# AdrienCorenflos/aux-ssm-samplers

Hardware: AMD Instinct MI355X
Metric: Gibbs sweeps/sec (aux-Kalman, parallel-in-time scan) (higher is better)
Workload: dtype f64; 1 GPU; C2: linear-Gaussian SSM T=65536 d=4 p=8, aux-Kalman sweep, parallel scan; chains_per_gpu=256, parallelism=chains x1 (independent, no collective)

## Files before the change

### aux_ssm_samplers_amd/csrc/api.hip

```cpp
#include <cstdarg>
#include <cstdlib>
#include <cstring>

#include "ctx.h"
#include "rng.h"

namespace ax {

static thread_local std::string g_err;
void set_error(const char* fmt, ...) {
    char buf[1024];
    va_list ap;
    va_start(ap, fmt);
    vsnprintf(buf, sizeof buf, fmt, ap);
    va_end(ap);
    g_err = buf;
}

int ws_reserve(auxssm_ctx* h, size_t bytes) {
    h->ws_off = 0;
    if (bytes <= h->ws_bytes) return AUXSSM_OK;
    if (h->ws) {
        AX_HIP(hipStreamSynchronize(h->stream));
        AX_HIP(hipFree(h->ws));
// ... 672 lines not shown
    if (aux_fly) {
        set_aux_fly(fa, c, 1, xA, epsauxA, uA);
        if (gen) fa.aux_gen = 1, fa.gen_k0 = keys[0], fa.gen_k1 = keys[1];
    }
    if (wide_shared) {
        const long long tot = (long long)T * P;
        hipLaunchKernelGGL((k_concat_carrier<R>), dim3((unsigned)((tot + 255) / 256)), dim3(256), 0, h->stream, T, D, P, cv(*c.yobs), carrier);
        fa.mask_ys = Arr{carrier, 0, (long long)P, 0, 1};
    }
    rc = ke->filter(h, fa, parallel, ell);
    if (rc) return rc;
    h->ws_off = mark;
    SampleArgs sa;
    fill_sample_args(sa, kd, D, cv(model->Fs), cv(model->Qs), cv(model->bs), msA, PsA, epsA, xpA, cm);
    sa.ps_shared = shared_mode ? 1 : 0;
    sa.ps_packed = ps_pack ? 1 : 0;
    if (gen) sa.eps_gen = 1, sa.gen_k0 = keys[2], sa.gen_k1 = keys[3];
    rc = se->sample(h, sa, parallel);
    if (rc) return rc;
    h->ws_off = mark;

    SweepLogpdfArgs la;
    fill_sweep_logpdf_args(la, c, kd, *model, cv(*c.yobs), xA, xpA, uA, aux_fly ? 1 : 0, epsauxA);
    rc = sl->run(h, la, sums);
    if (rc) return rc;
    h->ws_off = mark;
    launch_accept<R>(c, sums, ell, ell);
    if ((rc = launch_select<R>(h, C, T, D, (const int32_t*)c.accepted, xpA, xA, cm))) return rc;
    AX_HIP(hipGetLastError());
    return AUXSSM_OK;
}

template <typename R>
__global__ void k_fs_concat0(int C, int D, int PO, const R* __restrict__ xa, const R* __restrict__ xb, const int32_t* __restrict__ sel, const R* __restrict__ eps0, R shd,
                             const double* dptr, Arr yobs, R* __restrict__ u, R* __restrict__ ysc0) {
    if (dptr) shd = (R)dptr[1];
    const int P = D + PO;
    const int g = blockIdx.x * blockDim.x + threadIdx.x;
    if (g >= C * P) return;
    const int c = g % C, k = g / C;
    if (k < D) {
        const R* x = (sel && sel[c]) ? xb : xa;
        const R v = x[(long long)k * C + c] + shd * eps0[(long long)k * C + c];
        u[(long long)k * C + c] = v;
        ysc0[(long long)k * C + c] = v;
    } else {
        ysc0[(long long)k * C + c] = at<R>(yobs, 0, 0, 0)[k - D];
    }
}
template <typename R> __global__ void __launch_bounds__(256) k_fs_resolve(int C, const int32_t* __restrict__ sel, const R* __restrict__ xb, R* __restrict__ xa) {
    const int c = blockIdx.y * 256 + threadIdx.x;
    if (c >= C) return;
    const long long off = (long long)blockIdx.x * C + c;
    if (sel[c]) xa[off] = xb[off];
}
template <typename R>
__global__ void __launch_bounds__(256) k_fs_stats(int C, const int32_t* __restrict__ accepted, const int32_t* __restrict__ sel, const R* __restrict__ xa, const R* __restrict__ xb,
                                                   R* __restrict__ sq_jump, R* __restrict__ mean, R* __restrict__ sq_mean, long long iter) {
    const int c = blockIdx.y * 256 + threadIdx.x;
    if (c >= C) return;
    const long long off = (long long)blockIdx.x * C + c;
    const int s = sel[c], acc = accepted[c];
    const R xn = (s ? xb : xa)[off];
    const R xo = acc ? (s ? xa : xb)[off] : xn;
    const R it = (R)iter, dj = xn - xo;
    sq_jump[off] = fold_mean<R>(it, sq_jump[off], dj * dj);
    mean[off] = fold_mean<R>(it, mean[off], xn);
    sq_mean[off] = fold_mean<R>(it, sq_mean[off], xn * xn);
}
static const char* fused_refusal(const auxssm_ctx* h, const auxssm_dims* dims, const auxssm_lgssm* model, int parallel, int layout) {
    const int C = dims->C, T = dims->T, D = dims->dx, PO = dims->dy;
    if (layout != AUXSSM_LAYOUT_CHAIN_MINOR) return "the fused sweep takes the chain-minor layout";
    if (D > MAX_D || PO < 1 || PO > 4) return "the fused sweep is instantiated for dx <= 4, 1 <= dy <= 4";
    if (!parallel) return "the fused sweep is the parallel-in-time one";
    if (!h->share_model) return "AUXSSM_OPT_SHARE_MODEL is off";
    if (!prior_chain_shared(model)) return "the fused sweep needs chain-shared model parameters (chain stride 0)";
    if (C < 2 || (C % 2) != 0) return "the fused sweep pairs chains for its in-kernel draws: the chain count must be even";
    if (T < 64) return "the fused sweep needs T >= 64";
    return nullptr;
}
template <typename R> static int sweep_lg_concat_fused(const SweepCall& c) {
    auxssm_ctx* h = c.h;
    const auxssm_lgssm* model = c.model;
    const auxssm_arr* yobs = c.yobs;
    const double delta = c.delta;
    void *x = c.x, *x_alt = c.x_alt;
    const int C = c.dims->C, T = c.dims->T, D = c.dims->dx, PO = c.dims->dy, P = D + PO;
    const SweepLogpdfEntry* sl = sweep_logpdf_entry(c.dtype, D, PO);
    if (!sl || !sl->fused) {
        set_error("(dx=%d, dy=%d) has no fused sweep in this build", D, PO);
        return AUXSSM_ERR_UNSUPPORTED;
    }
    const KDims kd{C, T, 1};
    const size_t sR = sizeof(R), CT = (size_t)C * T;
    const size_t stage[4] = {(size_t)T * P * D * sR, (size_t)T * P * P * sR, (size_t)T * P * sR, (size_t)T * D * D * sR};
    R *u, *inc, *ysc0, *m0p, *eps0a, *eps0s;
    WsPlan ws;
    ws.add(u, CT * D * sR);
    ws.add(inc, CT * D * sR);
    ws.add(ysc0, (size_t)C * P * sR);
    ws.add(m0p, (size_t)C * D * sR);
    ws.add(eps0a, (size_t)C * D * sR);
    ws.add(eps0s, (size_t)C * D * sR);
    for (size_t b : stage) ws.after(b);
    ws.after(sl->fused_ws(h, kd));
    int rc = ws.reserve(h);
    if (rc) return rc;
    bool overlap = h->overlap_model_stage != 0 && !c.dptr;
    SweepEnd sweep_end{h};
    if (overlap) {
        const size_t need_side = sl->fused_ws(h, kd) + (size_t)(T + 64) * sR * ((size_t)P * D + (size_t)P * P + P + (size_t)D * D) + (4u << 20) +
                                 (size_t)(T + 2) * sR * (3 * (size_t)D * D + 2 * D + (size_t)PO * D + (size_t)PO * PO + 2 * PO);
        if ((rc = side_open(h, need_side))) return rc;
        overlap = h->side.open;
    }
    const bool tinv = obs_model_time_invariant(model);
    const int* memo = nullptr;
    struct MemoGuard {
        auxssm_ctx* h;
        int p = -1;
        bool ok = false;
        ~MemoGuard() { if (p >= 0 && !ok) h->side.memo_use[p] = -1; }
    } memo_guard{h};
    if (overlap) {
        SideScope sc(h);
        auxssm_ctx::SideStage& sd = h->side;
        const int p = sd.parity;
        MemoDesc md{};
        const auxssm_arr* srcs[9] = {&model->m0, &model->P0, &model->Fs, &model->Qs, &model->bs, &model->Hs, &model->Rs, &model->cs, yobs};
        const int recs[9] = {D, D * D, D * D, D * D, D, PO * D, PO * PO, PO, PO};
        const int nts[9] = {1, 1, T - 1, T - 1, T - 1, T, T, T, T};
        md.n = 9;
        md.off[0] = 0;
        bool plain = true;
        for (int q = 0; q < 9; ++q) {
// ... 9 lines not shown
        if (plain) {
            std::vector<unsigned char> key;
            auto put = [&](const void* v, size_t nb) { key.insert(key.end(), (const unsigned char*)v, (const unsigned char*)v + nb); };
            const int hdr[8] = {(int)sR, C, T, D, PO, c.nan_policy, 0, 0};
            put(hdr, sizeof(hdr));
            put(&delta, sizeof(delta));
            for (int q = 0; q < 9; ++q) put(srcs[q], sizeof(auxssm_arr));
            const bool chain_ok = sd.memo_use[p] == sd.uses[p] - 1 && sd.memo_key[p] == key;
            const unsigned gmemo = (unsigned)std::min<long long>(1024, (md.off[9] + 255) / 256);
            if (chain_ok) {
                hipLaunchKernelGGL(k_memo_set, dim3(1), dim3(1), 0, h->stream, rebuild, 0);
                hipLaunchKernelGGL((k_memo_check<R>), dim3(gmemo), dim3(256), 0, h->stream, md, (const R*)snap, rebuild);
            } else {
                hipLaunchKernelGGL(k_memo_set, dim3(1), dim3(1), 0, h->stream, rebuild, 1);
            }
            hipLaunchKernelGGL((k_memo_snap<R>), dim3(gmemo), dim3(256), 0, h->stream, md, snap, (const int*)rebuild);
            sd.memo_key[p] = std::move(key);
            sd.memo_use[p] = sd.uses[p];
            memo_guard.p = p;
            memo = rebuild;
        }
    }
    R *Hc, *Rc, *cc, *Ps;
    ConcatModel cmod;
    {
        SideScope sc(h);
        Hc = (R*)ws_take(h, stage[0]);
        Rc = (R*)ws_take(h, stage[1]);
        cc = (R*)ws_take(h, stage[2]);
        Ps = (R*)ws_take(h, stage[3]);
        if (!Hc || !Rc || !cc || !Ps) return AUXSSM_ERR_NOMEM;
        cmod = concat_model<R>(c, tinv, Hc, Rc, cc, memo, nullptr);
    }
    launch_rng_sweep<R>(h, c.keys, (long long)D * C, C, eps0a, eps0s, const_cast<void*>(c.u_acc));
    hipLaunchKernelGGL((k_fs_concat0<R>), dim3((unsigned)((C * P + 255) / 256)), dim3(256), 0, h->stream, C, D, PO, (const R*)x, (const R*)x_alt, (const int32_t*)c.sel,
                       (const R*)eps0a, (R)c.shd(), c.dptr, cv(*yobs), u, ysc0);
    FusedHost f{};
    const KDims k1{C, 1, 1};
    const Arr none{};
    sweep_filter_args(f.fa, cmod.d, cmod.g, cm_arr(ysc0, k1, P), cm_arr(m0p, k1, D), Arr{Ps, 0, (long long)D * D, 0, 1}, 1);
    f.fa.pblk = D;
    set_aux_fly(f.fa, c, 1, none, none, none);
    fill_sample_args(f.sa, kd, D, cv(model->Fs), cv(model->Qs), cv(model->bs), none, f.fa.Ps, none, none, 1);
    f.sa.ps_shared = 1;
    fill_sweep_logpdf_args(f.la, c, kd, *model, cv(*yobs), cm_arr(x, kd, D), cm_arr(x_alt, kd, D), cm_arr(u, kd, D), 0, none);
    f.memo = memo;
    f.xa = x; f.xb = x_alt; f.sel = c.sel; f.u = u; f.inc = inc; f.keys = c.keys; f.eps0s = eps0s; f.u_acc = c.u_acc; f.accepted = c.accepted; f.logs = c.logs;
    if (h->st_mean && (h->st_x != x || h->st_n != (long long)C * T * D || h->st_dtype != (sizeof(R) == 4 ? AUXSSM_F32 : AUXSSM_F64))) {
        set_error("running moments are attached to another state (x=%p, n=%lld, dtype=%d): detach them (auxssm_stats_attach with NULLs) "
                  "before sweeping a different state on this handle", h->st_x, h->st_n, h->st_dtype);
        return AUXSSM_ERR_ARG;
    }
    if ((rc = sl->fused(h, f))) return rc;
    if (!c.sel) {
        if ((rc = launch_select<R>(h, C, T, D, (const int32_t*)c.accepted, cm_arr(x_alt, kd, D), cm_arr(x, kd, D), 1))) return rc;
    } else if (h->st_mean) {
        ProfScope ps(h, AUXSSM_K_SELECT);
        const long long rows = (long long)T * D;
        hipLaunchKernelGGL((k_fs_stats<R>), dim3((unsigned)rows, (unsigned)((C + 255) / 256)), dim3(256), 0, h->stream, C, (const int32_t*)c.accepted, (const int32_t*)c.sel,
                           (const R*)x, (const R*)x_alt, (R*)h->st_sq_jump, (R*)h->st_mean, (R*)h->st_sq_mean, h->st_iter);
        ++h->st_iter;
    }
    AX_HIP(hipGetLastError());
    memo_guard.ok = true;
    return AUXSSM_OK;
}

template <typename R> AX_HD R sv_nan_to_num(R v) { return nan_to_num<R>(v); }
template <typename R>
// ... 962 lines not shown
```

### aux_ssm_samplers_amd/csrc/fused_shared.h

```cpp
#pragma once

struct FusedArgs {
    int C, T, E, nchunk;
    const void* xa;
    void* xb;
    const int32_t* sel;
    void* u;
    void* inc;
    const void* gain;
    const void* samp;
    const void* logt;
    const void* gpre;
    const void* m0p;
    void* agg_f; void* pre_f; void* agg_s; void* pre_s;
    Acc* pa;
    Acc* pe;
    void* pell;
    const Acc* clog;
    const int* nanrow;
    unsigned ka0, ka1, ks0, ks1;
    const void* eps0s;
    double delta, shd;
    const double* dptr;
    int nan_policy;
// ... 52 lines not shown
#pragma unroll
        for (int k = 0; k < D * D; ++k) G[k] = row[TS::oG + k];
        mm<R, D, D, D>(M, G, o);
#pragma unroll
        for (int k = 0; k < D * D; ++k) M[k] = o[k];
    }
#pragma unroll
    for (int k = 0; k < D * D; ++k) cprod[(long long)(a.nchunk - 1 - ch) * D * D + k] = M[k];
}

template <typename R, int D> __global__ void __launch_bounds__(TB_CM) k_fs_psi(FusedArgs a, const R* __restrict__ gpre, const R* __restrict__ fpre, R* __restrict__ ntab,
                                                                              R* __restrict__ psi) {
    if (memo_skip(a)) return;
    using TS = SampShared<R, D>;
    const int ch = blockIdx.x * TB_CM + threadIdx.x;
    if (ch >= a.nchunk) return;
    const int t0 = ch * a.E, tb = min(a.T, t0 + a.E);
    R Ps[D * D];
#pragma unroll
    for (int k = 0; k < D * D; ++k) Ps[k] = 0;
    for (int t = t0; t < tb; ++t) {
        const R* row = (const R*)a.samp + (long long)t * TS::NPAD;
        R M1[D * D], Ph[D * D], Gp[D * D], Nt[D * D], o[D * D];
#pragma unroll
        for (int k = 0; k < D * D; ++k) M1[k] = row[TS::oM + k], Ph[k] = fpre[(long long)t * D * D + k], Gp[k] = gpre[(long long)t * D * D + k];
        mm<R, D, D, D>(M1, Ph, Nt);
        mm<R, D, D, D>(Gp, Nt, o);
#pragma unroll
        for (int k = 0; k < D * D; ++k) ntab[(long long)t * D * D + k] = Nt[k], Ps[k] += o[k];
    }
#pragma unroll
    for (int k = 0; k < D * D; ++k) psi[(long long)ch * D * D + k] = Ps[k];
}
template <typename R, int D> __global__ void __launch_bounds__(256) k_fs_esfix(int C, int nchunk, const R* __restrict__ psi, const R* __restrict__ pre_f, R* __restrict__ agg_s) {
    const long long g = (long long)blockIdx.x * 256 + threadIdx.x;
    if (g >= (long long)C * nchunk) return;
    const int c = (int)(g / nchunk), ch = (int)(g % nchunk);
    if (ch == 0) return;
    R m[D], e[D], Ps[D * D];
    ldv<R, D>(pre_f + ((long long)c * nchunk + ch) * SampPre<R, D>::NPAD, m);
    R* q = agg_s + ((long long)c * nchunk + (nchunk - 1 - ch)) * SampPre<R, D>::NPAD;
    ldv<R, D>(q, e);
#pragma unroll
    for (int k = 0; k < D * D; ++k) Ps[k] = psi[(long long)ch * D * D + k];
#pragma unroll
    for (int i = 0; i < D; ++i) {
        R v = e[i];
#pragma unroll
        for (int k = 0; k < D; ++k) v += Ps[i * D + k] * m[k];
        e[i] = v;
    }
    stv<R, D>(q, e);
}

template <typename R, int D, int PO> struct FsRows {
    static constexpr int P = D + PO;
    using TL = LogShared<R, D, PO>;
    static constexpr int VEC = 16 / sizeof(R);
    static constexpr int pad(int n) { return (n + VEC - 1) / VEC * VEC; }
    static constexpr int cM = 0, cKc = D * D, cK = cKc + D, cM1 = cK + D * D, cGb = cM1 + D * D, cL = cGb + D, cGp = cL + symsize(D), cLg = cGp + D * D,
                         NC = pad(cLg + TL::N);
    static constexpr int eG = 0, eN = D * D, eL = 2 * D * D, NE = pad(eL + TL::N);
};
struct FsSrc { int tab, off; };
template <typename R, int D, int PO> __device__ __forceinline__ FsSrc fs_src_c(int k) {
    constexpr int P = D + PO;
    using F = FsRows<R, D, PO>; using TG = GainRow<R, D, P>; using TS = SampShared<R, D>; using TL = LogShared<R, D, PO>;
    if (k < F::cKc) return {0, TG::oM + k};
    if (k < F::cK) return {0, TG::oKc + (k - F::cKc)};
    if (k < F::cM1) { const int q = k - F::cK; return {0, TG::oK + (q / D) * P + (q % D)}; }
    if (k < F::cGb) return {1, TS::oM + (k - F::cM1)};
    if (k < F::cL) return {1, TS::oGb + (k - F::cGb)};
    if (k < F::cGp) {
        const int q = k - F::cL;
        int i = 0;
        while (lidx(i + 1, 0) <= q) ++i;
        return {1, TS::oL + i * D + (q - lidx(i, 0))};
    }
    if (k < F::cLg) return {3, k - F::cGp};
    if (k < F::cLg + TL::N) return {2, k - F::cLg};
    return {-1, 0};
}
template <typename R, int D, int PO> __device__ __forceinline__ FsSrc fs_src_e(int k) {
    using F = FsRows<R, D, PO>; using TS = SampShared<R, D>; using TL = LogShared<R, D, PO>;
    if (k < F::eN) return {1, TS::oG + k};
// ... 391 lines not shown
        R inc[D], ut[D], xp[D];
#pragma unroll
        for (int k = 0; k < D; ++k) inc[k] = incn[k], ut[k] = utn[k];
        if (t > t0) {
            const int tn = PK ? t - 1 : opaque_uniform(t - 1);
#pragma unroll
            for (int k = 0; k < D; ++k) incn[k] = ip[((long long)tn * D + k) * C], utn[k] = up[((long long)tn * D + k) * C];
        }
#pragma unroll
        for (int i = 0; i < D; ++i) {
            R v = inc[i];
#pragma unroll
            for (int k = 0; k < D; ++k) v += row[F::eN + i * D + k] * mst[k];
#pragma unroll
            for (int k = 0; k < D; ++k) v += row[F::eG + i * D + k] * h[k];
            xp[i] = v;
            xw[((long long)tu * D + i) * C] = v;
        }
        if (tu + 1 < a.T) {
            R w[3];
            if (fs_wave_any(fs_terms_fast<R, D, PO>(row + F::eL, h, xp, uq, inv_delta, cst, w))) fs_terms<R, D, PO>(a, row + F::eL, h, xp, uq, inv_delta, cst, w);
            v0 += (Acc)w[0];
            v1 += (Acc)w[1];
            v2 += (Acc)w[2];
        }
#pragma unroll
        for (int k = 0; k < D; ++k) h[k] = xp[k], uq[k] = ut[k];
    }
    a.pe[((long long)0 * C + c) * a.nchunk + ch] = v0;
    a.pe[((long long)1 * C + c) * a.nchunk + ch] = v1;
    a.pe[((long long)2 * C + c) * a.nchunk + ch] = v2;
}

template <typename R, int D, int PO> __global__ void __launch_bounds__(TB_ELEM) k_fs_head(SweepLogpdfArgs la, const void* xa, const void* xb, const int32_t* sel, R* __restrict__ head5) {
    resolve_step(la);
    const int c = blockIdx.x * TB_ELEM + threadIdx.x;
    if (c >= la.d.C) return;
    const bool sw = sel && sel[c];
    la.x.ptr = sw ? xb : xa;
    la.xp.ptr = sw ? xa : xb;
    R h5[5];
    body_sweep_logpdf_head<R, D, PO>(la, c, h5);
#pragma unroll
    for (int k = 0; k < 5; ++k) head5[(long long)k * la.d.C + c] = h5[k];
}

template <typename R, int D, int PO> __device__ __forceinline__ Acc fs_dropped_joint(const FusedArgs& a, const SweepLogpdfArgs& la, int c, const int32_t* sel) {
    Acc s = 0;
    const long long C = a.C;
    const R* xp = (const R*)((sel && sel[c]) ? a.xa : (const void*)a.xb) + c;
    const R* up = (const R*)a.u + c;
    const R inv_delta = (R)1 / (R)a.delta;
    const R cst = (R)-0.5 * (R)D * log_((R)(0.5 * a.delta)) - (R)(0.5 * LOG_2PI) * (R)D;
    for (int t = threadIdx.x; t < a.T; t += TB_ELEM) {
        R y[PO];
        rd<R, PO>(la.ys, c, t, 0, y);
        bool skip[PO], any = false;
#pragma unroll
        for (int k = 0; k < PO; ++k) skip[k] = !finite_(y[k]), any = any || skip[k];
        if (!any) continue;
        R H[PO * D], cv[PO], Rm[PO * PO], v[D], r[PO], q = 0;
        bool b = false;
        rd<R, PO * D>(la.Hs, c, t, 0, H);
        rd<R, PO>(la.cs, c, t, 0, cv);
        rd_upper<R, PO>(la.Rs, c, t, 0, Rm);
#pragma unroll
        for (int k = 0; k < D; ++k) {
            v[k] = xp[((long long)t * D + k) * C];
            const R d = up[((long long)t * D + k) * C] - v[k];
            b = b || !finite_(d);
            q += d * d;
        }
#pragma unroll
        for (int k = 0; k < PO; ++k) {
            R p = cv[k];
#pragma unroll
            for (int j = 0; j < D; ++j) p += H[k * D + j] * v[j];
            r[k] = y[k] - p;
        }
        s += (Acc)(b ? (R)0 : -q * inv_delta + cst) + (Acc)gauss_logpdf<R, PO>(r, Rm, skip);
    }
    return s;
}
template <typename R, int D, int PO> __global__ void __launch_bounds__(TB_ELEM) k_fs_accept(FusedArgs a, SweepLogpdfArgs lg, const R* __restrict__ head5, const R* __restrict__ ell0,
                                                                                            const R* __restrict__ u_acc, int32_t* __restrict__ accepted, R* __restrict__ logs,
                                                                                            int32_t* __restrict__ sel) {
    __shared__ Acc sh[TB_ELEM];
    fs_resolve(a);
    const int c = blockIdx.x;
    const long long C = a.C;
    bool any_dropped = false;
    if (a.nan_policy == 0) {
        R y0[PO];
        rd<R, PO>(lg.ys, c, 0, 0, y0);
        any_dropped = *a.nanrow != 0;
#pragma unroll
        for (int k = 0; k < PO; ++k) any_dropped = any_dropped || !finite_(y0[k]);
    }
    Acc tot[7] = {0, 0, 0, 0, 0, 0, 0};
    const R* pl = (const R*)a.pell + (long long)c * a.nchunk;
    for (int j = threadIdx.x; j < a.nchunk; j += TB_ELEM) {
#pragma unroll
        for (int k = 0; k < 3; ++k) tot[k] += a.pa[((long long)k * C + c) * a.nchunk + j], tot[3 + k] += a.pe[((long long)k * C + c) * a.nchunk + j];
        tot[6] += (Acc)pl[j];
    }
#pragma unroll
    for (int k = 0; k < 7; ++k) tot[k] = block_sum<Acc, TB_ELEM>(tot[k], sh);
    Acc dropped = 0;
    if (any_dropped) dropped = block_sum<Acc, TB_ELEM>(fs_dropped_joint<R, D, PO>(a, lg, c, sel), sh);
    if (threadIdx.x != 0) return;
    (void)ell0;
    const Acc jp_prop = tot[3] + (Acc)head5[0 * C + c], jp_rev = tot[0] + (Acc)head5[1 * C + c];
    const Acc ell = (jp_prop + dropped) - (tot[6] - *a.clog);
    const Acc lt_prop = tot[4] + (Acc)head5[2 * C + c], lt_rev = tot[1] + (Acc)head5[3 * C + c];
    const Acc corr = (tot[5] - tot[2]) + (Acc)head5[4 * C + c];
    const Acc lp_prop = jp_prop - ell, lp_rev = jp_rev - ell;
    Acc la = lt_prop - lt_rev;
    la += lp_rev - lp_prop;
    la -= corr;
    const Acc alpha = exp_(la != la ? la : min_(la, (Acc)0));
    const int acc = ((Acc)u_acc[c] < alpha) ? 1 : 0;
    accepted[c] = acc;
    if (sel) sel[c] ^= acc;
    if (logs) {
        logs[c * 5 + 0] = (R)la;
        logs[c * 5 + 1] = (R)lp_prop;
        logs[c * 5 + 2] = (R)lp_rev;
        logs[c * 5 + 3] = (R)lt_prop;
        logs[c * 5 + 4] = (R)lt_rev;
    }
}

inline int fs_pack(int C, int* cp_out) {
    int cp = 2;
    while (cp < C) cp <<= 1;
    *cp_out = cp;
    constexpr int lanes = 256;
    if (cp > lanes / 2) return 1;
    const int pack = lanes / cp;
    constexpr int cap = 8;
    return pack > cap ? cap : pack;
}
inline int fs_chunk_len(const auxssm_ctx* h, int C, int T) {
    constexpr int waves = 10;
    const long long stiles = (C + TB_CM - 1) / TB_CM;
    long long want = (long long)h->num_cu * 4 * waves / stiles;
    if (want < 1) want = 1;
    long long E = (T + want - 1) / want;
    if (E < 16) E = 16;
    if (E > 32) E = 32;
    if (C >= 1024) E = 64;
    else if (C >= 96) E = 32;
    if (E > T) E = T > 2 ? T : 2;
    return (int)E;
}
template <typename R, int D, int PO> size_t fused_ws(const auxssm_ctx* h, const KDims& d) {
    constexpr int P = D + PO;
    const int E = fs_chunk_len(h, d.C, d.T), nchunk = (d.T + E - 1) / E;
    size_t b = 0;
    b += (size_t)d.C * nchunk * (4 * SampPre<R, D>::NPAD * sizeof(R) + 6 * sizeof(Acc) + sizeof(R)) + 16 * 256;
    b += (size_t)d.C * (5 + 1 + D) * sizeof(R) + 4 * 256;
    b += filter_ws<R, D, P>(h, KDims{1, d.T, 1}, 1);
    b += (size_t)d.T * (SampShared<R, D>::NPAD + LogShared<R, D, PO>::NPAD + (size_t)D * D) * sizeof(R) + (size_t)2 * nchunk * D * D * sizeof(R) + 10 * 256 + ((size_t)d.T / 256 + 2) * sizeof(Acc);
    b += (size_t)d.T * (FsRows<R, D, PO>::NC + FsRows<R, D, PO>::NE + 2 * (size_t)D * D) * sizeof(R) + (size_t)nchunk * D * D * sizeof(R) + 8 * 256;
    return b;
}
template <typename R, int D, int PO> int run_fused_shared(auxssm_ctx* h, FusedHost& f) {
    constexpr int P = D + PO;
    const int C = f.fa.d.C, T = f.fa.d.T, n = T - 1;
    FusedArgs a{};
    a.C = C; a.T = T;
    a.E = fs_chunk_len(h, C, T);
    a.nchunk = (T + a.E - 1) / a.E;
    a.pack = fs_pack(C, &a.cp);
    {
        using FR = FsRows<R, D, PO>;
        constexpr int NMAX = FR::NC > FR::NE ? FR::NC : FR::NE;
        while (a.pack > 1 && (size_t)a.pack * fs_pk_block<R, NMAX>(a.E) * sizeof(R) + FsNormTabSel<R>::BYTES > (size_t)128 * 1024) a.pack >>= 1;
    }
    a.xa = f.xa; a.xb = f.xb; a.sel = f.sel; a.u = f.u; a.inc = f.inc;
    a.ka0 = f.keys[0]; a.ka1 = f.keys[1]; a.ks0 = f.keys[2]; a.ks1 = f.keys[3];
    a.eps0s = f.eps0s;
    a.delta = f.la.delta; a.shd = f.la.shd; a.dptr = f.la.dptr; a.nan_policy = f.la.nan_policy;
    a.memo = f.memo;
    f.fa.memo = f.sa.memo = f.la.memo = f.memo;
    R *cprod_f, *cprod_s, *rows_c, *rows_e, *psi;
    {
        {
            const int rc = build_gain_table<R, D, P>(h, f.fa);
            if (rc) return rc;
        }
        SideScope side(h);
        f.sa.tab = ws_take(h, (size_t)T * SampShared<R, D>::NPAD * sizeof(R));
        f.la.tab = ws_take(h, (size_t)n * LogShared<R, D, PO>::NPAD * sizeof(R));
        R* gpre = (R*)ws_take(h, (size_t)T * D * D * sizeof(R));
        cprod_f = (R*)ws_take(h, (size_t)a.nchunk * D * D * sizeof(R));
        cprod_s = (R*)ws_take(h, (size_t)a.nchunk * D * D * sizeof(R));
        rows_c = (R*)ws_take(h, (size_t)T * FsRows<R, D, PO>::NC * sizeof(R));
        rows_e = (R*)ws_take(h, (size_t)T * FsRows<R, D, PO>::NE * sizeof(R));
        R* fpre = (R*)ws_take(h, (size_t)T * D * D * sizeof(R));
        R* ntab = (R*)ws_take(h, (size_t)T * D * D * sizeof(R));
        psi = (R*)ws_take(h, (size_t)a.nchunk * D * D * sizeof(R));
        const int nclb = (T + 255) / 256;
        Acc* clog = (Acc*)ws_take(h, 256 + (size_t)nclb * sizeof(Acc));
        if (!f.sa.tab || !f.la.tab || !gpre || !cprod_f || !cprod_s || !rows_c || !rows_e || !fpre || !ntab || !psi || !clog) return AUXSSM_ERR_NOMEM;
        a.clog = clog;
        int* nanrow = (int*)(clog + 16);
        a.nanrow = nanrow;
        a.gain = f.fa.tab; a.samp = f.sa.tab; a.logt = f.la.tab; a.gpre = gpre;
        {
            ProfScope ps(h, AUXSSM_K_SAMPLE_INIT);
            hipLaunchKernelGGL((k_sample_shared_tab<R, D>), dim3((T + TB_ELEM - 1) / TB_ELEM), dim3(TB_ELEM), 0, h->stream, f.sa);
            hipLaunchKernelGGL((k_fs_clog_part<R, D>), dim3(nclb), dim3(256), 0, h->stream, T, (const R*)f.sa.tab, clog + 32, f.memo);
            hipLaunchKernelGGL((k_fs_clog_sum<D>), dim3(1), dim3(256), 0, h->stream, T, nclb, (const Acc*)(clog + 32), clog, nanrow, f.memo);
            hipLaunchKernelGGL((k_sweep_logpdf_tab<R, D, PO>), dim3((n + TB_ELEM - 1) / TB_ELEM), dim3(TB_ELEM), 0, h->stream, f.la);
            hipLaunchKernelGGL((k_fs_fprod<R, D, P>), dim3((a.nchunk + TB_CM - 1) / TB_CM), dim3(TB_CM), 0, h->stream, a, cprod_f, fpre);
            hipLaunchKernelGGL((k_fs_gpre<R, D>), dim3((a.nchunk + TB_CM - 1) / TB_CM), dim3(TB_CM), 0, h->stream, a, gpre, cprod_s);
            hipLaunchKernelGGL((k_fs_psi<R, D>), dim3((a.nchunk + TB_CM - 1) / TB_CM), dim3(TB_CM), 0, h->stream, a, (const R*)gpre, (const R*)fpre, ntab, psi);
            {
                using F = FsRows<R, D, PO>;
                const long long nmax = (long long)T * (F::NC > F::NE ? F::NC : F::NE);
                hipLaunchKernelGGL((k_fs_rows<R, D, PO>), dim3((unsigned)((nmax + 255) / 256), 2), dim3(256), 0, h->stream, a, (const R*)ntab, rows_c, rows_e, nanrow);
            }
        }
    }
    {
        const int rc = side_close(h);
        if (rc) return rc;
    }
    a.memo = nullptr;
    f.fa.memo = f.sa.memo = f.la.memo = nullptr;
    const size_t npre = (size_t)C * a.nchunk * SampPre<R, D>::NPAD * sizeof(R);
    a.agg_f = ws_take(h, npre); a.pre_f = ws_take(h, npre); a.agg_s = ws_take(h, npre); a.pre_s = ws_take(h, npre);
    a.pa = (Acc*)ws_take(h, (size_t)3 * C * a.nchunk * sizeof(Acc));
    a.pe = (Acc*)ws_take(h, (size_t)3 * C * a.nchunk * sizeof(Acc));
    a.pell = ws_take(h, (size_t)C * a.nchunk * sizeof(R));
    R* head5 = (R*)ws_take(h, (size_t)5 * C * sizeof(R));
    f.fa.ell0 = ws_take(h, (size_t)C * sizeof(R));
    if (!a.agg_f || !a.pre_f || !a.agg_s || !a.pre_s || !a.pa || !a.pe || !a.pell || !head5 || !f.fa.ell0) return AUXSSM_ERR_NOMEM;
    a.m0p = f.fa.ms.ptr;
    f.fa.t0_keep_ps = 1;
    hipLaunchKernelGGL((k_filter_t0<R, D, P>), dim3((C + TB_ELEM - 1) / TB_ELEM), dim3(TB_ELEM), 0, h->stream, f.fa);
    using F = FsRows<R, D, PO>;
    const int TBF = C >= 256 ? 256 : (C + 63) / 64 * 64;
    const unsigned grid = (unsigned)a.nchunk * (unsigned)((C + TBF - 1) / TBF);
    const unsigned grid_pk = (unsigned)((a.nchunk + a.pack - 1) / a.pack);
    const size_t lds = (size_t)TB_AGGS * SampElem<R, D>::NPAD * sizeof(R);
    if (a.pack > 1) {
        const size_t lds_ac = (size_t)a.pack * fs_pk_block<R, F::NC>(a.E) * sizeof(R) + FsNormTabSel<R>::BYTES;
        if (lds_ac > 64 * 1024) AX_HIP(hipFuncSetAttribute((const void*)k_fs_ac<R, D, PO, true>, hipFuncAttributeMaxDynamicSharedMemorySize, (int)lds_ac));
        ProfScope ps(h, AUXSSM_K_FILTER_SCAN);
        hipLaunchKernelGGL((k_fs_ac<R, D, PO, true>), dim3(grid_pk), dim3(a.pack * a.cp), lds_ac, h->stream, a, (const R*)rows_c);
    } else {
        const size_t lds_ac = (size_t)a.E * F::NC * sizeof(R) + FsNormTabSel<R>::BYTES;
        if (lds_ac > 64 * 1024) AX_HIP(hipFuncSetAttribute((const void*)k_fs_ac<R, D, PO>, hipFuncAttributeMaxDynamicSharedMemorySize, (int)lds_ac));
        ProfScope ps(h, AUXSSM_K_FILTER_SCAN);
        hipLaunchKernelGGL((k_fs_ac<R, D, PO>), dim3(grid), dim3(TBF), lds_ac, h->stream, a, (const R*)rows_c);
    }
    {
        ProfScope ps(h, AUXSSM_K_SAMPLE_SCAN);
        hipLaunchKernelGGL((k_aff_aggs<R, D>), dim3(C), dim3(TB_AGGS), lds, h->stream, ScanBufs{a.agg_f, a.pre_f}, (const R*)cprod_f, a.nchunk);
        hipLaunchKernelGGL((k_fs_esfix<R, D>), dim3((unsigned)(((long long)C * a.nchunk + 255) / 256)), dim3(256), 0, h->stream, C, a.nchunk, (const R*)psi, (const R*)a.pre_f,
                           (R*)a.agg_s);
        hipLaunchKernelGGL((k_aff_aggs<R, D>), dim3(C), dim3(TB_AGGS), lds, h->stream, ScanBufs{a.agg_s, a.pre_s}, (const R*)cprod_s, a.nchunk);
    }
    {
        ProfScope ps(h, AUXSSM_K_LOGPDF);
        if (a.pack > 1) {
            const size_t lds_e = (size_t)a.pack * fs_pk_block<R, F::NE>(a.E) * sizeof(R);
            if (lds_e > 64 * 1024) AX_HIP(hipFuncSetAttribute((const void*)k_fs_e<R, D, PO, true>, hipFuncAttributeMaxDynamicSharedMemorySize, (int)lds_e));
            hipLaunchKernelGGL((k_fs_e<R, D, PO, true>), dim3(grid_pk), dim3(a.pack * a.cp), lds_e, h->stream, a, (const R*)rows_e);
        } else
            hipLaunchKernelGGL((k_fs_e<R, D, PO>), dim3(grid), dim3(TBF), (size_t)a.E * F::NE * sizeof(R), h->stream, a, (const R*)rows_e);
    }
    {
        ProfScope ps(h, AUXSSM_K_SELECT);
        hipLaunchKernelGGL((k_fs_head<R, D, PO>), dim3((C + TB_ELEM - 1) / TB_ELEM), dim3(TB_ELEM), 0, h->stream, f.la, f.xa, (const void*)f.xb, (const int32_t*)f.sel, head5);
        hipLaunchKernelGGL((k_fs_accept<R, D, PO>), dim3(C), dim3(TB_ELEM), 0, h->stream, a, f.la, (const R*)head5, (const R*)f.fa.ell0, (const R*)f.u_acc, f.accepted,
                           (R*)f.logs, f.sel);
    }
    AX_HIP(hipGetLastError());
    return AUXSSM_OK;
}
```

Measured before the change: 278,400 sweeps/s.

## Fuse sweep prologue RNG, merge chunk scans with shared prefix tables, inline head terms

Replaces the separate RNG launch and concat kernel with one prologue kernel that draws normals and uniforms in place. The two per-chain aggregate scans and the esfix pass become a single kernel. It uses Kogge-Stone level tables of chunk-transition products, built once per model in k_fs_scantab, so per-chain scans do matrix-vector work instead of matrix-matrix. The head-term kernel is folded into the accept kernel, and the seven block reductions are batched into one. The T threshold is also lowered, and there is a risk of changed RNG stream mapping and larger LDS and workspace use.

```diff
diff --git a/aux_ssm_samplers_amd/csrc/api.hip b/aux_ssm_samplers_amd/csrc/api.hip
--- a/aux_ssm_samplers_amd/csrc/api.hip
+++ b/aux_ssm_samplers_amd/csrc/api.hip
@@ -728,20 +728,49 @@
 }
 
 template <typename R>
-__global__ void k_fs_concat0(int C, int D, int PO, const R* __restrict__ xa, const R* __restrict__ xb, const int32_t* __restrict__ sel, const R* __restrict__ eps0, R shd,
-                             const double* dptr, Arr yobs, R* __restrict__ u, R* __restrict__ ysc0) {
-    if (dptr) shd = (R)dptr[1];
-    const int P = D + PO;
-    const int g = blockIdx.x * blockDim.x + threadIdx.x;
-    if (g >= C * P) return;
-    const int c = g % C, k = g / C;
-    if (k < D) {
-        const R* x = (sel && sel[c]) ? xb : xa;
-        const R v = x[(long long)k * C + c] + shd * eps0[(long long)k * C + c];
-        u[(long long)k * C + c] = v;
-        ysc0[(long long)k * C + c] = v;
+__global__ void __launch_bounds__(256) k_fs_prologue(uint32_t a0, uint32_t a1, uint32_t b0, uint32_t b1, uint32_t c0, uint32_t c1, int C, int D, int PO, unsigned g1, unsigned g2,
+                                                      const R* __restrict__ xa, const R* __restrict__ xb, const int32_t* __restrict__ sel, R shd, const double* dptr, Arr yobs,
+                                                      R* __restrict__ u, R* __restrict__ ysc0, R* __restrict__ eps0s, R* __restrict__ u_acc) {
+    const unsigned blk = blockIdx.x;
+    const long long n = (long long)D * C;
+    if (blk < 2 * g1) {
+        const bool second = blk >= g1;
+        const long long i = (long long)(second ? blk - g1 : blk) * blockDim.x + threadIdx.x;
+        if (2 * i >= n) return;
+        uint32_t x0, x1;
+        stream_counter(0, (unsigned long long)i, x0, x1);
+        threefry2x32(second ? b0 : a0, second ? b1 : a1, x0, x1);
+        R z0, z1;
+        bits_to_normal2<R>(x0, x1, z0, z1);
+        if (second) {
+            eps0s[2 * i] = z0;
+            if (2 * i + 1 < n) eps0s[2 * i + 1] = z1;
+            return;
+        }
+        if (dptr) shd = (R)dptr[1];
+        const R z[2] = {z0, z1};
+#pragma unroll
+        for (int q = 0; q < 2; ++q) {
+            const long long g = 2 * i + q;
+            if (g >= n) break;
+            const int c = (int)(g % C);
+            const R* x = (sel && sel[c]) ? xb : xa;
+            const R v = x[g] + shd * z[q];
+            u[g] = v;
+            ysc0[g] = v;
+        }
+    } else if (blk < 2 * g1 + g2) {
+        const long long i = (long long)(blk - 2 * g1) * blockDim.x + threadIdx.x;
+        if (2 * i >= C) return;
+        R u0, u1;
+        stream_uniform2<R>(c0, c1, 0, (unsigned long long)i, u0, u1);
+        u_acc[2 * i] = u0;
+        if (2 * i + 1 < C) u_acc[2 * i + 1] = u1;
     } else {
-        ysc0[(long long)k * C + c] = at<R>(yobs, 0, 0, 0)[k - D];
+        const long long g = (long long)(blk - 2 * g1 - g2) * blockDim.x + threadIdx.x;
+        if (g >= (long long)C * PO) return;
+        const int k = (int)(g / C);
+        ysc0[n + g] = at<R>(yobs, 0, 0, 0)[k];
     }
 }
 template <typename R> __global__ void __launch_bounds__(256) k_fs_resolve(int C, const int32_t* __restrict__ sel, const R* __restrict__ xb, R* __restrict__ xa) {
@@ -772,7 +801,7 @@
     if (!h->share_model) return "AUXSSM_OPT_SHARE_MODEL is off";
     if (!prior_chain_shared(model)) return "the fused sweep needs chain-shared model parameters (chain stride 0)";
     if (C < 2 || (C % 2) != 0) return "the fused sweep pairs chains for its in-kernel draws: the chain count must be even";
-    if (T < 64) return "the fused sweep needs T >= 64";
+    if (T < 16) return "the fused sweep needs T >= 16";
     return nullptr;
 }
 template <typename R> static int sweep_lg_concat_fused(const SweepCall& c) {
@@ -790,13 +819,12 @@
     const KDims kd{C, T, 1};
     const size_t sR = sizeof(R), CT = (size_t)C * T;
     const size_t stage[4] = {(size_t)T * P * D * sR, (size_t)T * P * P * sR, (size_t)T * P * sR, (size_t)T * D * D * sR};
-    R *u, *inc, *ysc0, *m0p, *eps0a, *eps0s;
+    R *u, *inc, *ysc0, *m0p, *eps0s;
     WsPlan ws;
     ws.add(u, CT * D * sR);
     ws.add(inc, CT * D * sR);
     ws.add(ysc0, (size_t)C * P * sR);
     ws.add(m0p, (size_t)C * D * sR);
-    ws.add(eps0a, (size_t)C * D * sR);
     ws.add(eps0s, (size_t)C * D * sR);
     for (size_t b : stage) ws.after(b);
     ws.after(sl->fused_ws(h, kd));
@@ -872,9 +900,13 @@
         if (!Hc || !Rc || !cc || !Ps) return AUXSSM_ERR_NOMEM;
         cmod = concat_model<R>(c, tinv, Hc, Rc, cc, memo, nullptr);
     }
-    launch_rng_sweep<R>(h, c.keys, (long long)D * C, C, eps0a, eps0s, const_cast<void*>(c.u_acc));
-    hipLaunchKernelGGL((k_fs_concat0<R>), dim3((unsigned)((C * P + 255) / 256)), dim3(256), 0, h->stream, C, D, PO, (const R*)x, (const R*)x_alt, (const int32_t*)c.sel,
-                       (const R*)eps0a, (R)c.shd(), c.dptr, cv(*yobs), u, ysc0);
+    {
+        const long long n0 = (long long)D * C;
+        const unsigned g1 = (unsigned)(((n0 + 1) / 2 + 255) / 256), g2 = (unsigned)(((C + 1) / 2 + 255) / 256), g3 = (unsigned)(((long long)C * PO + 255) / 256);
+        ProfScope ps(h, AUXSSM_K_RNG);
+        hipLaunchKernelGGL((k_fs_prologue<R>), dim3(2 * g1 + g2 + g3), dim3(256), 0, h->stream, c.keys[0], c.keys[1], c.keys[2], c.keys[3], c.keys[4], c.keys[5], C, D, PO, g1, g2,
+                           (const R*)x, (const R*)x_alt, (const int32_t*)c.sel, (R)c.shd(), c.dptr, cv(*yobs), u, ysc0, eps0s, (R*)const_cast<void*>(c.u_acc));
+    }
     FusedHost f{};
     const KDims k1{C, 1, 1};
     const Arr none{};
diff --git a/aux_ssm_samplers_amd/csrc/fused_shared.h b/aux_ssm_samplers_amd/csrc/fused_shared.h
--- a/aux_ssm_samplers_amd/csrc/fused_shared.h
+++ b/aux_ssm_samplers_amd/csrc/fused_shared.h
@@ -108,25 +108,161 @@
 #pragma unroll
     for (int k = 0; k < D * D; ++k) psi[(long long)ch * D * D + k] = Ps[k];
 }
-template <typename R, int D> __global__ void __launch_bounds__(256) k_fs_esfix(int C, int nchunk, const R* __restrict__ psi, const R* __restrict__ pre_f, R* __restrict__ agg_s) {
-    const long long g = (long long)blockIdx.x * 256 + threadIdx.x;
-    if (g >= (long long)C * nchunk) return;
-    const int c = (int)(g / nchunk), ch = (int)(g % nchunk);
-    if (ch == 0) return;
-    R m[D], e[D], Ps[D * D];
-    ldv<R, D>(pre_f + ((long long)c * nchunk + ch) * SampPre<R, D>::NPAD, m);
-    R* q = agg_s + ((long long)c * nchunk + (nchunk - 1 - ch)) * SampPre<R, D>::NPAD;
-    ldv<R, D>(q, e);
-#pragma unroll
-    for (int k = 0; k < D * D; ++k) Ps[k] = psi[(long long)ch * D * D + k];
-#pragma unroll
-    for (int i = 0; i < D; ++i) {
-        R v = e[i];
-#pragma unroll
-        for (int k = 0; k < D; ++k) v += Ps[i * D + k] * m[k];
-        e[i] = v;
-    }
-    stv<R, D>(q, e);
+constexpr int FS_LVL = 8;
+static_assert((1 << FS_LVL) == TB_AGGS, "one table level per Kogge-Stone level of the aggregate scan");
+template <typename R, int D> struct FsScan {
+    static constexpr int VEC = 16 / sizeof(R);
+    static constexpr int GP = (D * D + VEC - 1) / VEC * VEC;
+    static constexpr size_t TAB = (size_t)FS_LVL * TB_AGGS * D * D;
+};
+template <typename R, int D> __global__ void __launch_bounds__(TB_AGGS) k_fs_scantab(FusedArgs a, const R* __restrict__ cprod_f, const R* __restrict__ cprod_s,
+                                                                                      R* __restrict__ ltab_f, R* __restrict__ ltab_s) {
+    if (memo_skip(a)) return;
+    constexpr int GP = FsScan<R, D>::GP;
+    __shared__ __attribute__((aligned(16))) R lds[TB_AGGS * GP];
+    const R* cprod = blockIdx.x ? cprod_s : cprod_f;
+    R* ltab = blockIdx.x ? ltab_s : ltab_f;
+    const int tid = threadIdx.x, nchunk = a.nchunk;
+    const int E2 = (nchunk + TB_AGGS - 1) / TB_AGGS;
+    const int j0 = min(nchunk, tid * E2), j1 = min(nchunk, j0 + E2);
+    R G[D * D];
+#pragma unroll
+    for (int k = 0; k < D * D; ++k) G[k] = (k / D == k % D) ? (R)1 : (R)0;
+    if (j0 < j1) ldv<R, D * D>(cprod + (long long)j0 * D * D, G);
+    for (int j = j0 + 1; j < j1; ++j) {
+        R cur[D * D], o[D * D];
+        ldv<R, D * D>(cprod + (long long)j * D * D, cur);
+        mm<R, D, D, D>(cur, G, o);
+#pragma unroll
+        for (int k = 0; k < D * D; ++k) G[k] = o[k];
+    }
+    int lvl = 0;
+    for (int off = 1; off < TB_AGGS; off <<= 1, ++lvl) {
+        R* out = ltab + ((long long)lvl * TB_AGGS + tid) * D * D;
+#pragma unroll
+        for (int k = 0; k < D * D; ++k) out[k] = G[k], lds[tid * GP + k] = G[k];
+        __syncthreads();
+        R left[D * D];
+        if (tid >= off) {
+#pragma unroll
+            for (int k = 0; k < D * D; ++k) left[k] = lds[(tid - off) * GP + k];
+        }
+        __syncthreads();
+        if (tid >= off) {
+            R o[D * D];
+            mm<R, D, D, D>(G, left, o);
+#pragma unroll
+            for (int k = 0; k < D * D; ++k) G[k] = o[k];
+        }
+    }
+}
+template <typename R, int D, class LD1, class LD3>
+__device__ __forceinline__ void fs_scan_e(int nchunk, const R* __restrict__ cprod, const R* __restrict__ ltab, R* __restrict__ pre, R* lds, LD1 ld1, LD3 ld3) {
+    constexpr int NP = SampPre<R, D>::NPAD;
+    const int tid = threadIdx.x;
+    const int E2 = (nchunk + TB_AGGS - 1) / TB_AGGS;
+    const int j0 = min(nchunk, tid * E2), j1 = min(nchunk, j0 + E2);
+    R e[D];
+#pragma unroll
+    for (int k = 0; k < D; ++k) e[k] = 0;
+    if (j0 < j1) ld1(j0, e);
+    {
+        R Gn[D * D], en[D];
+        if (j0 + 1 < j1) ldv<R, D * D>(cprod + (long long)(j0 + 1) * D * D, Gn), ld1(j0 + 1, en);
+        for (int j = j0 + 1; j < j1; ++j) {
+            R Gc[D * D], ec[D], t[D];
+#pragma unroll
+            for (int k = 0; k < D * D; ++k) Gc[k] = Gn[k];
+#pragma unroll
+            for (int k = 0; k < D; ++k) ec[k] = en[k];
+            if (j + 1 < j1) ldv<R, D * D>(cprod + (long long)(j + 1) * D * D, Gn), ld1(j + 1, en);
+            mv<R, D, D>(Gc, e, t);
+#pragma unroll
+            for (int i = 0; i < D; ++i) e[i] = t[i] + ec[i];
+        }
+    }
+    R Ln[D * D];
+#pragma unroll
+    for (int k = 0; k < D * D; ++k) Ln[k] = 0;
+    if (tid >= 1) ldv<R, D * D>(ltab + (long long)tid * D * D, Ln);
+#pragma unroll
+    for (int lvl = 0; lvl < FS_LVL; ++lvl) {
+        const int off = 1 << lvl;
+        R L[D * D];
+#pragma unroll
+        for (int k = 0; k < D * D; ++k) L[k] = Ln[k];
+        if (lvl + 1 < FS_LVL && tid >= 2 * off) ldv<R, D * D>(ltab + ((long long)(lvl + 1) * TB_AGGS + tid) * D * D, Ln);
+        stv<R, D>(lds + tid * NP, e);
+        __syncthreads();
+        R left[D];
+        if (tid >= off) ldv<R, D>(lds + (tid - off) * NP, left);
+        __syncthreads();
+        if (tid >= off) {
+            R t[D];
+            mv<R, D, D>(L, left, t);
+#pragma unroll
+            for (int i = 0; i < D; ++i) e[i] = t[i] + e[i];
+        }
+    }
+    stv<R, D>(lds + tid * NP, e);
+    __syncthreads();
+    R p[D];
+#pragma unroll
+    for (int k = 0; k < D; ++k) p[k] = 0;
+    if (tid > 0) ldv<R, D>(lds + (tid - 1) * NP, p);
+    __syncthreads();
+    {
+        R Gn[D * D], en[D];
+        if (j0 + 1 < j1) ldv<R, D * D>(cprod + (long long)j0 * D * D, Gn), ld3(j0, en);
+        for (int j = j0; j < j1; ++j) {
+            stv<R, D>(pre + (long long)j * NP, p);
+            if (j + 1 < j1) {
+                R Gc[D * D], ec[D], t[D];
+#pragma unroll
+                for (int k = 0; k < D * D; ++k) Gc[k] = Gn[k];
+#pragma unroll
+                for (int k = 0; k < D; ++k) ec[k] = en[k];
+                if (j + 2 < j1) ldv<R, D * D>(cprod + (long long)(j + 1) * D * D, Gn), ld3(j + 1, en);
+                mv<R, D, D>(Gc, p, t);
+#pragma unroll
+                for (int i = 0; i < D; ++i) p[i] = t[i] + ec[i];
+            }
+        }
+    }
+}
+template <typename R, int D> __global__ void __launch_bounds__(TB_AGGS) k_fs_scans(FusedArgs a, const R* __restrict__ cprod_f, const R* __restrict__ ltab_f,
+                                                                                    const R* __restrict__ cprod_s, const R* __restrict__ ltab_s, const R* __restrict__ psi) {
+    constexpr int NP = SampPre<R, D>::NPAD;
+    __shared__ __attribute__((aligned(16))) R lds[TB_AGGS * NP];
+    const int nchunk = a.nchunk;
+    const long long base = (long long)blockIdx.x * nchunk * NP;
+    const R* agg_f = (const R*)a.agg_f + base;
+    R* pre_f = (R*)a.pre_f + base;
+    R* agg_s = (R*)a.agg_s + base;
+    R* pre_s = (R*)a.pre_s + base;
+    auto ldf = [&](int j, R* e) { ldv<R, D>(agg_f + (long long)j * NP, e); };
+    fs_scan_e<R, D>(nchunk, cprod_f, ltab_f, pre_f, lds, ldf, ldf);
+    __syncthreads();
+    auto lds1 = [&](int j, R* e) {
+        const int ch = nchunk - 1 - j;
+        R* q = agg_s + (long long)j * NP;
+        ldv<R, D>(q, e);
+        if (ch == 0) return;
+        R m[D], Ps[D * D];
+        ldv<R, D>(pre_f + (long long)ch * NP, m);
+#pragma unroll
+        for (int k = 0; k < D * D; ++k) Ps[k] = psi[(long long)ch * D * D + k];
+#pragma unroll
+        for (int i = 0; i < D; ++i) {
+            R v = e[i];
+#pragma unroll
+            for (int k = 0; k < D; ++k) v += Ps[i * D + k] * m[k];
+            e[i] = v;
+        }
+        stv<R, D>(q, e);
+    };
+    auto lds3 = [&](int j, R* e) { ldv<R, D>(agg_s + (long long)j * NP, e); };
+    fs_scan_e<R, D>(nchunk, cprod_s, ltab_s, pre_s, lds, lds1, lds3);
 }
 
 template <typename R, int D, int PO> struct FsRows {
@@ -584,19 +720,23 @@
     a.pe[((long long)2 * C + c) * a.nchunk + ch] = v2;
 }
 
-template <typename R, int D, int PO> __global__ void __launch_bounds__(TB_ELEM) k_fs_head(SweepLogpdfArgs la, const void* xa, const void* xb, const int32_t* sel, R* __restrict__ head5) {
-    resolve_step(la);
-    const int c = blockIdx.x * TB_ELEM + threadIdx.x;
-    if (c >= la.d.C) return;
-    const bool sw = sel && sel[c];
-    la.x.ptr = sw ? xb : xa;
-    la.xp.ptr = sw ? xa : xb;
-    R h5[5];
-    body_sweep_logpdf_head<R, D, PO>(la, c, h5);
-#pragma unroll
-    for (int k = 0; k < 5; ++k) head5[(long long)k * la.d.C + c] = h5[k];
-}
-
+template <int TB> __device__ __forceinline__ void fs_block_sum7(Acc* v, Acc* sh) {
+    const int tid = threadIdx.x;
+#pragma unroll
+    for (int k = 0; k < 7; ++k) sh[k * TB + tid] = v[k];
+    __syncthreads();
+#pragma unroll
+    for (int off = TB / 2; off > 0; off >>= 1) {
+        if (tid < off) {
+#pragma unroll
+            for (int k = 0; k < 7; ++k) sh[k * TB + tid] += sh[k * TB + tid + off];
+        }
+        __syncthreads();
+    }
+#pragma unroll
+    for (int k = 0; k < 7; ++k) v[k] = sh[k * TB];
+    __syncthreads();
+}
 template <typename R, int D, int PO> __device__ __forceinline__ Acc fs_dropped_joint(const FusedArgs& a, const SweepLogpdfArgs& la, int c, const int32_t* sel) {
     Acc s = 0;
     const long long C = a.C;
@@ -634,13 +774,26 @@
     }
     return s;
 }
-template <typename R, int D, int PO> __global__ void __launch_bounds__(TB_ELEM) k_fs_accept(FusedArgs a, SweepLogpdfArgs lg, const R* __restrict__ head5, const R* __restrict__ ell0,
+template <typename R, int D, int PO> __global__ void __launch_bounds__(TB_ELEM) k_fs_accept(FusedArgs a, SweepLogpdfArgs lg, const R* __restrict__ ell0,
                                                                                             const R* __restrict__ u_acc, int32_t* __restrict__ accepted, R* __restrict__ logs,
                                                                                             int32_t* __restrict__ sel) {
-    __shared__ Acc sh[TB_ELEM];
+    __shared__ Acc sh[7 * TB_ELEM];
+    __shared__ R head5[5];
+    static_assert(TB_ELEM > 64, "the t = 0 terms are formed by a lane of the second wave");
     fs_resolve(a);
     const int c = blockIdx.x;
     const long long C = a.C;
+    if (threadIdx.x == 64) {
+        SweepLogpdfArgs la = lg;
+        resolve_step(la);
+        const bool sw = sel && sel[c];
+        la.x.ptr = sw ? (const void*)a.xb : a.xa;
+        la.xp.ptr = sw ? a.xa : (const void*)a.xb;
+        R h5[5];
+        body_sweep_logpdf_head<R, D, PO>(la, c, h5);
+#pragma unroll
+        for (int k = 0; k < 5; ++k) head5[k] = h5[k];
+    }
     bool any_dropped = false;
     if (a.nan_policy == 0) {
         R y0[PO];
@@ -656,16 +809,15 @@
         for (int k = 0; k < 3; ++k) tot[k] += a.pa[((long long)k * C + c) * a.nchunk + j], tot[3 + k] += a.pe[((long long)k * C + c) * a.nchunk + j];
         tot[6] += (Acc)pl[j];
     }
-#pragma unroll
-    for (int k = 0; k < 7; ++k) tot[k] = block_sum<Acc, TB_ELEM>(tot[k], sh);
+    fs_block_sum7<TB_ELEM>(tot, sh);
     Acc dropped = 0;
     if (any_dropped) dropped = block_sum<Acc, TB_ELEM>(fs_dropped_joint<R, D, PO>(a, lg, c, sel), sh);
     if (threadIdx.x != 0) return;
     (void)ell0;
-    const Acc jp_prop = tot[3] + (Acc)head5[0 * C + c], jp_rev = tot[0] + (Acc)head5[1 * C + c];
+    const Acc jp_prop = tot[3] + (Acc)head5[0], jp_rev = tot[0] + (Acc)head5[1];
     const Acc ell = (jp_prop + dropped) - (tot[6] - *a.clog);
-    const Acc lt_prop = tot[4] + (Acc)head5[2 * C + c], lt_rev = tot[1] + (Acc)head5[3 * C + c];
-    const Acc corr = (tot[5] - tot[2]) + (Acc)head5[4 * C + c];
+    const Acc lt_prop = tot[4] + (Acc)head5[2], lt_rev = tot[1] + (Acc)head5[3];
+    const Acc corr = (tot[5] - tot[2]) + (Acc)head5[4];
     const Acc lp_prop = jp_prop - ell, lp_rev = jp_rev - ell;
     Acc la = lt_prop - lt_rev;
     la += lp_rev - lp_prop;
@@ -715,6 +867,7 @@
     b += filter_ws<R, D, P>(h, KDims{1, d.T, 1}, 1);
     b += (size_t)d.T * (SampShared<R, D>::NPAD + LogShared<R, D, PO>::NPAD + (size_t)D * D) * sizeof(R) + (size_t)2 * nchunk * D * D * sizeof(R) + 10 * 256 + ((size_t)d.T / 256 + 2) * sizeof(Acc);
     b += (size_t)d.T * (FsRows<R, D, PO>::NC + FsRows<R, D, PO>::NE + 2 * (size_t)D * D) * sizeof(R) + (size_t)nchunk * D * D * sizeof(R) + 8 * 256;
+    b += 2 * FsScan<R, D>::TAB * sizeof(R) + 2 * 256;
     return b;
 }
 template <typename R, int D, int PO> int run_fused_shared(auxssm_ctx* h, FusedHost& f) {
@@ -736,7 +889,7 @@
     a.delta = f.la.delta; a.shd = f.la.shd; a.dptr = f.la.dptr; a.nan_policy = f.la.nan_policy;
     a.memo = f.memo;
     f.fa.memo = f.sa.memo = f.la.memo = f.memo;
-    R *cprod_f, *cprod_s, *rows_c, *rows_e, *psi;
+    R *cprod_f, *cprod_s, *rows_c, *rows_e, *psi, *ltab_f, *ltab_s;
     {
         {
             const int rc = build_gain_table<R, D, P>(h, f.fa);
@@ -753,9 +906,11 @@
         R* fpre = (R*)ws_take(h, (size_t)T * D * D * sizeof(R));
         R* ntab = (R*)ws_take(h, (size_t)T * D * D * sizeof(R));
         psi = (R*)ws_take(h, (size_t)a.nchunk * D * D * sizeof(R));
+        ltab_f = (R*)ws_take(h, FsScan<R, D>::TAB * sizeof(R));
+        ltab_s = (R*)ws_take(h, FsScan<R, D>::TAB * sizeof(R));
         const int nclb = (T + 255) / 256;
         Acc* clog = (Acc*)ws_take(h, 256 + (size_t)nclb * sizeof(Acc));
-        if (!f.sa.tab || !f.la.tab || !gpre || !cprod_f || !cprod_s || !rows_c || !rows_e || !fpre || !ntab || !psi || !clog) return AUXSSM_ERR_NOMEM;
+        if (!f.sa.tab || !f.la.tab || !gpre || !cprod_f || !cprod_s || !rows_c || !rows_e || !fpre || !ntab || !psi || !ltab_f || !ltab_s || !clog) return AUXSSM_ERR_NOMEM;
         a.clog = clog;
         int* nanrow = (int*)(clog + 16);
         a.nanrow = nanrow;
@@ -768,6 +923,7 @@
             hipLaunchKernelGGL((k_sweep_logpdf_tab<R, D, PO>), dim3((n + TB_ELEM - 1) / TB_ELEM), dim3(TB_ELEM), 0, h->stream, f.la);
             hipLaunchKernelGGL((k_fs_fprod<R, D, P>), dim3((a.nchunk + TB_CM - 1) / TB_CM), dim3(TB_CM), 0, h->stream, a, cprod_f, fpre);
             hipLaunchKernelGGL((k_fs_gpre<R, D>), dim3((a.nchunk + TB_CM - 1) / TB_CM), dim3(TB_CM), 0, h->stream, a, gpre, cprod_s);
+            hipLaunchKernelGGL((k_fs_scantab<R, D>), dim3(2), dim3(TB_AGGS), 0, h->stream, a, (const R*)cprod_f, (const R*)cprod_s, ltab_f, ltab_s);
             hipLaunchKernelGGL((k_fs_psi<R, D>), dim3((a.nchunk + TB_CM - 1) / TB_CM), dim3(TB_CM), 0, h->stream, a, (const R*)gpre, (const R*)fpre, ntab, psi);
             {
                 using F = FsRows<R, D, PO>;
@@ -787,9 +943,8 @@
     a.pa = (Acc*)ws_take(h, (size_t)3 * C * a.nchunk * sizeof(Acc));
     a.pe = (Acc*)ws_take(h, (size_t)3 * C * a.nchunk * sizeof(Acc));
     a.pell = ws_take(h, (size_t)C * a.nchunk * sizeof(R));
-    R* head5 = (R*)ws_take(h, (size_t)5 * C * sizeof(R));
     f.fa.ell0 = ws_take(h, (size_t)C * sizeof(R));
-    if (!a.agg_f || !a.pre_f || !a.agg_s || !a.pre_s || !a.pa || !a.pe || !a.pell || !head5 || !f.fa.ell0) return AUXSSM_ERR_NOMEM;
+    if (!a.agg_f || !a.pre_f || !a.agg_s || !a.pre_s || !a.pa || !a.pe || !a.pell || !f.fa.ell0) return AUXSSM_ERR_NOMEM;
     a.m0p = f.fa.ms.ptr;
     f.fa.t0_keep_ps = 1;
     hipLaunchKernelGGL((k_filter_t0<R, D, P>), dim3((C + TB_ELEM - 1) / TB_ELEM), dim3(TB_ELEM), 0, h->stream, f.fa);
@@ -797,7 +952,6 @@
     const int TBF = C >= 256 ? 256 : (C + 63) / 64 * 64;
     const unsigned grid = (unsigned)a.nchunk * (unsigned)((C + TBF - 1) / TBF);
     const unsigned grid_pk = (unsigned)((a.nchunk + a.pack - 1) / a.pack);
-    const size_t lds = (size_t)TB_AGGS * SampElem<R, D>::NPAD * sizeof(R);
     if (a.pack > 1) {
         const size_t lds_ac = (size_t)a.pack * fs_pk_block<R, F::NC>(a.E) * sizeof(R) + FsNormTabSel<R>::BYTES;
         if (lds_ac > 64 * 1024) AX_HIP(hipFuncSetAttribute((const void*)k_fs_ac<R, D, PO, true>, hipFuncAttributeMaxDynamicSharedMemorySize, (int)lds_ac));
@@ -811,10 +965,7 @@
     }
     {
         ProfScope ps(h, AUXSSM_K_SAMPLE_SCAN);
-        hipLaunchKernelGGL((k_aff_aggs<R, D>), dim3(C), dim3(TB_AGGS), lds, h->stream, ScanBufs{a.agg_f, a.pre_f}, (const R*)cprod_f, a.nchunk);
-        hipLaunchKernelGGL((k_fs_esfix<R, D>), dim3((unsigned)(((long long)C * a.nchunk + 255) / 256)), dim3(256), 0, h->stream, C, a.nchunk, (const R*)psi, (const R*)a.pre_f,
-                           (R*)a.agg_s);
-        hipLaunchKernelGGL((k_aff_aggs<R, D>), dim3(C), dim3(TB_AGGS), lds, h->stream, ScanBufs{a.agg_s, a.pre_s}, (const R*)cprod_s, a.nchunk);
+        hipLaunchKernelGGL((k_fs_scans<R, D>), dim3(C), dim3(TB_AGGS), 0, h->stream, a, (const R*)cprod_f, (const R*)ltab_f, (const R*)cprod_s, (const R*)ltab_s, (const R*)psi);
     }
     {
         ProfScope ps(h, AUXSSM_K_LOGPDF);
@@ -827,8 +978,7 @@
     }
     {
         ProfScope ps(h, AUXSSM_K_SELECT);
-        hipLaunchKernelGGL((k_fs_head<R, D, PO>), dim3((C + TB_ELEM - 1) / TB_ELEM), dim3(TB_ELEM), 0, h->stream, f.la, f.xa, (const void*)f.xb, (const int32_t*)f.sel, head5);
-        hipLaunchKernelGGL((k_fs_accept<R, D, PO>), dim3(C), dim3(TB_ELEM), 0, h->stream, a, f.la, (const R*)head5, (const R*)f.fa.ell0, (const R*)f.u_acc, f.accepted,
+        hipLaunchKernelGGL((k_fs_accept<R, D, PO>), dim3(C), dim3(TB_ELEM), 0, h->stream, a, f.la, (const R*)f.fa.ell0, (const R*)f.u_acc, f.accepted,
                            (R*)f.logs, f.sel);
     }
     AX_HIP(hipGetLastError());
```

Result: no change. 276,900 sweeps/s (-0.6%).
